# OpenDriveLab/OccNet

Measured on AMD Instinct MI355X. Metric: nuScenes samples/sec (6-cam 900x1600 -> 200x200x16 voxels), higher is better.
Workload: dtype f32 hot path (GEMM operands bf16x3-split, SCA value rows q16 block floating point) + bf16 backbone; 1 GPU; bevformer_base_occ forward: 6x(3x928x1600) images -> ResNet-50+FPN -> 4 BEVFormer layers (TSA+SCA+FFN) -> lifter + 2xConv3d decoder -> 200x200x16 voxels x (17 logits + 2 flow); history_frames=0, mode=infer, scope=e2e, input=resident-f32, samples_per_gpu=1, global_batch=1, parallelism=dp1, step_graph=False, linear_precision=bf16x3, backbone_dtype=bf16

## Files before the change

include/occnet_amd.h:

```cpp
#ifndef OCCNET_AMD_H_
#define OCCNET_AMD_H_

#include <stdint.h>

#ifdef __cplusplus
extern "C" {
#endif

#define OCC_OK 0
#define OCC_E_INVALID (-1)
#define OCC_E_LAUNCH (-2)
#define OCC_E_UNSUPPORTED (-3)

int occ_abi_version(void);
const char* occ_last_error(void);
int occ_selftest_fdiv_f32(const float* a, const float* d, float* q, int64_t n, void* stream);


int occ_ms_deform_attn_forward_f32(const float* value, const int64_t* spatial_shapes,
                                   const int64_t* level_start_index, const float* sampling_loc,
                                   const float* attn_weight, float* out, int B, int S, int M, int D,
                                   int L, int Lq, int P, int im2col_step, void* stream);

int occ_ms_deform_attn_backward_f32(const float* value, const int64_t* spatial_shapes,
// ... 121 lines not shown

int occ_sca_prep_forward_f32(const float* proj, int64_t proj_batch_stride, int proj_ld, const int64_t* row_to_query,
                             const float* ref_rb, const int64_t* spatial_shapes, float* loc, float* attn, int B,
                             int64_t R, int M, int L, int P, int Z, void* stream);
int occ_sca_prep_backward_f32(const float* grad_loc, const float* grad_attn, const float* attn,
                              const int64_t* query_to_rows, int Kq, const int64_t* spatial_shapes, float* dproj,
                              int proj_ld, int B, int64_t R, int64_t Q, int M, int L, int P, void* stream);

int occ_rows_gather_sum_f32(const float* x, int64_t x_batch_stride, const int64_t* index, int K, float* out, int B,
                            int64_t rows_out, int64_t rows_in, int F, void* stream);

int64_t occ_linear_wgrad_workspace_bytes(int M, int N, int K);
int occ_linear_wgrad_bf16x3_f32(const float* dy, int64_t lddy, const float* x, int64_t ldx, float* dw, float* db,
                                void* workspace, int64_t workspace_bytes, int M, int N, int K, void* stream);

int64_t occ_conv3d_wgrad_workspace_bytes(int B, int Z, int Y, int X, int Cin);
int occ_conv3d_wgrad_bf16x3_f32(const float* dy_pad, const float* x_pad, float* dw, void* workspace,
                                int64_t workspace_bytes, int B, int Z, int Y, int X, int Cin, void* stream);

int occ_bias_act_nhwc_bf16(void* x, const float* bias, const void* residual, int64_t rows, int C, int relu,
                           void* stream);

int64_t occ_bias_act_bwd_partial_floats(int64_t rows, int C);
int occ_bias_act_bwd_nhwc_bf16(const void* grad_y, const void* y, void* g, float* partial, float* bias_grad,
                               int64_t rows, int C, int relu, void* stream);

int occ_conv_bn_fold_fwd_f32(const float* weight, const float* gamma, const float* beta, const float* rstd,
                             const float* mean_rstd, float* w_folded, void* w_folded_bf16_nhwc, float* bias, int Cout,
                             int Cin, int KH, int KW, void* stream);
int occ_conv_bn_fold_bwd_f32(const void* grad_w_bf16, int64_t stride_o, int64_t stride_i, int64_t stride_h, int64_t stride_w,
                             const float* weight, const float* gamma, const float* rstd, const float* mean_rstd,
                             const float* grad_bias, float* grad_weight, float* grad_gamma, int Cout, int Cin, int KH, int KW,
                             void* stream);

unsigned occ_ln_dropout_hash(unsigned index, unsigned seed_lo, unsigned seed_hi);
int64_t occ_dropout_add_ln_bwd_partial_floats(int64_t rows, int C);
int occ_dropout_add_ln_fwd_f32(const float* x, const float* residual, const float* gamma, const float* beta, float eps,
                               float p_drop, uint64_t seed, float* z, float* y, float* stats, int64_t rows, int C,
                               void* stream);
int occ_dropout_add_ln_bwd_f32(const float* grad_y, const float* z, const float* stats, const float* gamma, float p_drop,
                               uint64_t seed, float* grad_x, float* grad_residual, float* partial, float* grad_gamma_beta,
                               int64_t rows, int C, void* stream);

int occ_value_proj_bf16_f32(int n_segments, const void* const* a, const int64_t* lda, const int64_t* rows,
                            const int64_t* rows_per_group, const int64_t* out_row0,
                            const float* const* group_bias, int bias_groups, const void* weight_packed,
                            float* out, int64_t ldo, int K, int N, int64_t out_group_rows, void* stream);
int occ_value_proj_bf16_f16pairs(int n_segments, const void* const* a, const int64_t* lda, const int64_t* rows,
                            const int64_t* rows_per_group, const int64_t* out_row0,
                            const float* const* group_bias, int bias_groups, const void* weight_packed,
                            void* out, int64_t ldo, int K, int N, int64_t out_group_rows, const float* out_scale,
                            void* stream);
int occ_value_proj_bf16_q16pairs(int n_segments, const void* const* a, const int64_t* lda, const int64_t* rows,
                            const int64_t* rows_per_group, const int64_t* out_row0,
                            const float* const* group_bias, int bias_groups, const void* weight_packed,
                            void* out, int64_t ldo, int K, int N, int64_t out_group_rows, const float* out_scale,
                            void* stream);

int occ_value_range_scale_bf16(int n_segments, const void* const* a, const int64_t* lda, const int64_t* rows, int K,
                               int n_planes, const float* row_l1, const float* bias_max, float* scale_out,
                               uint32_t* work, void* stream);
int occ_value_range_scale_from_amax(const uint32_t* amax8, int n_planes, const float* row_l1, const float* bias_max,
                                    float* scale_out, void* stream);

int occ_value_proj_bf16_planes(int n_segments, const void* const* a, const int64_t* lda, const int64_t* rows,
                               const int64_t* rows_per_group, const int64_t* out_row0,
                               const float* const* group_bias, int bias_groups, const void* weight_packed, void* out,
                               int out_f16, int64_t ldo, int K, int n_planes, int plane_cols, int64_t plane_stride,
                               int64_t out_group_rows, const float* out_scale, void* stream);

int occ_stem_conv7x7_pool_f32_bf16(const float* x, const void* weight_frag, const float* bias, void* out,
                                   int batch, int H, int W, void* stream);
int occ_stem_conv7x7_pool_u8_bf16(const uint8_t* x, const void* weight_frag, const float* bias, void* out,
                                  int batch, int Hs, int Ws, int H, int W, const float* mean,
                                  const float* std, int to_rgb, void* stream);

int occ_bias_relu_maxpool_nhwc_bf16(const void* y, const float* bias, void* out, int batch, int H, int W, int C,
                                    void* stream);

int occ_conv1x1_nhwc_bf16(const void* x, const void* weight, const float* bias, const void* residual,
                          void* out, int batch, int Hin, int Win, int Cin, int Cout, int stride, int relu,
                          int residual_upsample2, void* stream);

int occ_conv3x3_pack_weight_bf16(const float* weight, void* packed, int Cout, int Cin, void* stream);
int occ_conv3x3_nhwc_bf16(const void* x, const void* weight_packed, const float* bias, void* out, int batch,
                          int H, int W, int Cin, int Cout, int stride, int relu, void* stream);
int occ_conv3x3_nhwc_bf16_amax(const void* x, const void* weight_packed, const float* bias, void* out, int batch,
                               int H, int W, int Cin, int Cout, int stride, int relu, uint32_t* amax8, void* stream);
int occ_conv3x3_nhwc_bf16_variant(const void* x, const void* weight_packed, const float* bias, void* out, int batch,
                                  int H, int W, int Cin, int Cout, int stride, int relu, uint32_t* amax8, int variant,
                                  void* stream);

int occ_mfma_pack_b_frag_bf16(const float* weight, void* packed, int N, int K, void* stream);

int occ_bottleneck64_nhwc_bf16(const void* x, const void* w1_frag, const float* b1, const void* w2_frag,
                               const float* b2, const void* w3_frag, const float* b3, void* out, int batch,
                               int H, int W, int Cin, int downsample, void* stream);

#ifdef __cplusplus
}
#endif
#endif
```

occnet_amd/csrc/conv1x1_nhwc_bf16.hip:

```cpp
#include "common.h"

namespace occ {

typedef float f32x16 __attribute__((ext_vector_type(16)));
typedef __bf16 bf16x8 __attribute__((ext_vector_type(8)));


__device__ __forceinline__ float c1_bf16_to_f32(unsigned short h) { return __uint_as_float((unsigned)h << 16); }

template <int NT, int RT>
__global__ __launch_bounds__(256) void conv1x1_nhwc_bf16_kernel(
    const uint4* __restrict__ x, const uint4* __restrict__ w, const float* __restrict__ bias,
    const unsigned short* __restrict__ residual, unsigned short* __restrict__ out, long M, int N, int K,
    int Hin, int Win, int Hout, int Wout, int stride, int relu, int res_up) {
  constexpr int KC = 32, kCLD = KC * 2 + 16, PC = KC / 8;
  constexpr int BM = 32 * RT, BN = 128 * NT, WR = 32 * NT, OLD = BN + 4;
  constexpr int AP = BM * PC / 256;
  constexpr int A_BYTES = BM * kCLD;
  constexpr int STAGE_BYTES = 2 * A_BYTES, OUT_BYTES = 32 * OLD * 4;
  __shared__ __attribute__((aligned(16))) char lds[STAGE_BYTES > OUT_BYTES ? STAGE_BYTES : OUT_BYTES];
  const int tid = threadIdx.x, lane = tid & 63, wave = tid >> 6;
  const int vi = lane & 31, kb = lane >> 5;
  const long m0 = (long)blockIdx.x * BM;
  const int n0 = blockIdx.y * BN;
  const int KQ = K / 8;
  const int NT32 = N / 32;

  f32x16 acc[RT][NT];
#pragma unroll
  for (int rt = 0; rt < RT; ++rt)
#pragma unroll
    for (int t = 0; t < NT; ++t)
#pragma unroll
      for (int r = 0; r < 16; ++r) acc[rt][t][r] = 0.f;

  static_assert(AP >= 1 && AP <= 2 && NT <= 2, "staging register budget");
  long aofs[AP];
  int adst[AP];
#pragma unroll
  for (int ap = 0; ap < AP; ++ap) {
    const int j = tid + 256 * ap;
    const int row = j / PC, piece = j % PC;
    long m = m0 + row;
    if (m >= M) m = M - 1;
    long pix = m;
    if (stride != 1) {
      const long hw = (long)Hout * Wout;
      const long n = m / hw, rem = m % hw;
      const int yo = (int)(rem / Wout), xo = (int)(rem % Wout);
      pix = (n * Hin + (long)yo * stride) * Win + (long)xo * stride;
    }
    aofs[ap] = pix * KQ + piece;
    adst[ap] = row * kCLD + piece * 16;
  }
  const int nt0 = min((n0 + wave * WR) / 32, NT32 - 1), nt1 = min((n0 + wave * WR) / 32 + (NT - 1), NT32 - 1);
  const long wl0 = (long)nt0 * 64 + lane, wl1 = (long)nt1 * 64 + lane;
  uint4 va0_0, va1_0, va0_1, va1_1;
  uint4 wa0_0, wa1_0, wb0_0, wb1_0, wa0_1, wa1_1, wb0_1, wb1_1, wa0_2, wa1_2, wb0_2, wb1_2;
#define OCC_C1_ISSUE_A(S, K0)                                                                     \
  {                                                                                               \
    const long kq = (K0) / 8;                                                                     \
    va0_##S = x[aofs[0] + kq];                                                                    \
    if (AP > 1) va1_##S = x[aofs[AP > 1 ? 1 : 0] + kq];                                           \
  }
#define OCC_C1_ISSUE_W(S, K0)                                                                     \
  {                                                                                               \
    const long k0 = (long)((K0) / 16) * NT32 * 64, k1 = k0 + (long)NT32 * 64;                     \
    wa0_##S = w[k0 + wl0]; wb0_##S = w[k1 + wl0];                                                 \
    if (NT > 1) { wa1_##S = w[k0 + wl1]; wb1_##S = w[k1 + wl1]; }                                 \
  }
#define OCC_C1_STEP(SA, SW, SWN, BUF, K_NEXT)                                                     \
  {                                                                                               \
    char* sA = lds + (BUF) * A_BYTES;                                                             \
    *reinterpret_cast<uint4*>(sA + adst[0]) = va0_##SA;                                           \
    if (AP > 1) *reinterpret_cast<uint4*>(sA + adst[AP > 1 ? 1 : 0]) = va1_##SA;                  \
    __syncthreads();                 \
    OCC_C1_ISSUE_A(SA, K_NEXT)                                                                    \
    OCC_C1_ISSUE_W(SWN, K_NEXT)                                                                   \
    bf16x8 af[RT][2];                                                                             \
    _Pragma("unroll") for (int rt = 0; rt < RT; ++rt)                                             \
      _Pragma("unroll") for (int ks = 0; ks < 2; ++ks)                                            \
        af[rt][ks] = *reinterpret_cast<const bf16x8*>(sA + (rt * 32 + vi) * kCLD + ks * 32 + kb * 16); \
// ... 1 lines not shown
      acc[rt][0] = __builtin_amdgcn_mfma_f32_32x32x16_bf16(af[rt][0], __builtin_bit_cast(bf16x8, wa0_##SW), acc[rt][0], 0, 0, 0); \
      if (NT > 1) acc[rt][NT - 1] = __builtin_amdgcn_mfma_f32_32x32x16_bf16(af[rt][0], __builtin_bit_cast(bf16x8, wa1_##SW), acc[rt][NT - 1], 0, 0, 0); \
    }                                                                                             \
    _Pragma("unroll") for (int rt = 0; rt < RT; ++rt) {                                           \
      acc[rt][0] = __builtin_amdgcn_mfma_f32_32x32x16_bf16(af[rt][1], __builtin_bit_cast(bf16x8, wb0_##SW), acc[rt][0], 0, 0, 0); \
      if (NT > 1) acc[rt][NT - 1] = __builtin_amdgcn_mfma_f32_32x32x16_bf16(af[rt][1], __builtin_bit_cast(bf16x8, wb1_##SW), acc[rt][NT - 1], 0, 0, 0); \
    }                                                                                             \
  }

  const int NCHK = K / KC;
  const int rot = (int)((blockIdx.x * 5u + blockIdx.y * 3u) % (unsigned)NCHK);
#define OCC_C1_K(CI) ((((CI) < NCHK ? (CI) : NCHK - 1) + rot) % NCHK * KC)
  OCC_C1_ISSUE_A(0, OCC_C1_K(0))
  OCC_C1_ISSUE_W(0, OCC_C1_K(0))
  OCC_C1_ISSUE_A(1, OCC_C1_K(1))
  OCC_C1_ISSUE_W(1, OCC_C1_K(1))
  for (int ci = 0; ci < NCHK; ci += 6) {
    OCC_C1_STEP(0, 0, 2, 0, OCC_C1_K(ci + 2))
    if (ci + 1 < NCHK) OCC_C1_STEP(1, 1, 0, 1, OCC_C1_K(ci + 3))
    if (ci + 2 < NCHK) OCC_C1_STEP(0, 2, 1, 0, OCC_C1_K(ci + 4))
    if (ci + 3 < NCHK) OCC_C1_STEP(1, 0, 2, 1, OCC_C1_K(ci + 5))
    if (ci + 4 < NCHK) OCC_C1_STEP(0, 1, 0, 0, OCC_C1_K(ci + 6))
    if (ci + 5 < NCHK) OCC_C1_STEP(1, 2, 1, 1, OCC_C1_K(ci + 7))
  }
#undef OCC_C1_K
#undef OCC_C1_STEP
#undef OCC_C1_ISSUE_A
#undef OCC_C1_ISSUE_W

  const int c = lane * 4;
  const bool col_live = c < BN && n0 + c < N;
  float4 bv = make_float4(0.f, 0.f, 0.f, 0.f);
  if (col_live) bv = *reinterpret_cast<const float4*>(bias + n0 + c);
  float* sO = reinterpret_cast<float*>(lds);
#pragma unroll
  for (int rt = 0; rt < RT; ++rt) {
    __syncthreads();
#pragma unroll
    for (int t = 0; t < NT; ++t)
#pragma unroll
      for (int r = 0; r < 16; ++r)
        sO[((r & 3) + 8 * (r >> 2) + 4 * kb) * OLD + (wave * NT + t) * 32 + vi] = acc[rt][t][r];
    __syncthreads();
    uint2 rv[8];
#pragma unroll
    for (int rr = 0; rr < 8; ++rr) {
      long m = m0 + rt * 32 + wave * 8 + rr;
      if (m >= M) m = M - 1;
      rv[rr] = make_uint2(0u, 0u);
      if (residual != nullptr && col_live) {
        long rrow = m;
        if (res_up) {
          const long hw = (long)Hout * Wout;
          const long n = m / hw, rem = m - n * hw;
          const int yo = (int)(rem / Wout), xo = (int)(rem - (long)yo * Wout);
          rrow = (n * (Hout >> 1) + (yo >> 1)) * (Wout >> 1) + (xo >> 1);
        }
        rv[rr] = *reinterpret_cast<const uint2*>(residual + rrow * N + n0 + c);
      }
    }
#pragma unroll
    for (int rr = 0; rr < 8; ++rr) {
      const int row = wave * 8 + rr;
      const long m = m0 + rt * 32 + row;
      if (m < M && col_live) {
        float4 v = *reinterpret_cast<const float4*>(sO + row * OLD + c);
        v.x += bv.x; v.y += bv.y; v.z += bv.z; v.w += bv.w;
        v.x += c1_bf16_to_f32((unsigned short)(rv[rr].x & 0xffffu));
        v.y += c1_bf16_to_f32((unsigned short)(rv[rr].x >> 16));
        v.z += c1_bf16_to_f32((unsigned short)(rv[rr].y & 0xffffu));
        v.w += c1_bf16_to_f32((unsigned short)(rv[rr].y >> 16));
        if (relu) {
          v.x = fmaxf(v.x, 0.f); v.y = fmaxf(v.y, 0.f); v.z = fmaxf(v.z, 0.f); v.w = fmaxf(v.w, 0.f);
        }
        const uint2 o = make_uint2(pack_bf16x2_rne(v.x, v.y), pack_bf16x2_rne(v.z, v.w));
        *reinterpret_cast<uint2*>(out + m * N + n0 + c) = o;
      }
    }
  }
}

}

extern "C" int occ_conv1x1_nhwc_bf16(const void* x, const void* weight, const float* bias,
                                     const void* residual, void* out, int batch, int Hin, int Win,
                                     int Cin, int Cout, int stride, int relu, int residual_upsample2,
                                     void* stream) {
  using namespace occ;
  OCC_CHECK_ARG(x && weight && bias && out, "conv1x1_nhwc_bf16: null pointer argument");
  OCC_CHECK_ARG(batch > 0 && Hin > 0 && Win > 0 && Cin > 0 && Cout > 0 && stride > 0,
                "conv1x1_nhwc_bf16: bad dimension");
  if (Cin % 32 || Cout % 32) {
    set_error("conv1x1_nhwc_bf16: no kernel for Cin=%d Cout=%d (need Cin %% 32 == 0, Cout %% 32 == 0)", Cin,
              Cout);
    return OCC_E_UNSUPPORTED;
  }
  const int Hout = (Hin - 1) / stride + 1, Wout = (Win - 1) / stride + 1;
  OCC_CHECK_ARG(!residual_upsample2 || (residual && Hout % 2 == 0 && Wout % 2 == 0),
                "conv1x1_nhwc_bf16: an upsampled residual needs even output sizes (exact x2 nearest upsampling)");
  const long M = (long)batch * Hout * Wout;
  hipStream_t st = reinterpret_cast<hipStream_t>(stream);
#define OCC_C1_LAUNCH(NTT, RTT, BNN)                                                                \
  hipLaunchKernelGGL((conv1x1_nhwc_bf16_kernel<NTT, RTT>),                                          \
                     dim3((unsigned)((M + 32 * RTT - 1) / (32 * RTT)), (unsigned)((Cout + BNN - 1) / BNN)), \
                     dim3(256), 0, st, reinterpret_cast<const uint4*>(x),                           \
                     reinterpret_cast<const uint4*>(weight), bias,                                  \
                     reinterpret_cast<const unsigned short*>(residual),                             \
                     reinterpret_cast<unsigned short*>(out), M, Cout, Cin, Hin, Win, Hout, Wout, stride, relu,  \
                     residual_upsample2)
  if (Cout <= 128) OCC_C1_LAUNCH(1, 2, 128); else OCC_C1_LAUNCH(2, 2, 256);
#undef OCC_C1_LAUNCH
  OCC_CHECK_LAUNCH("conv1x1_nhwc_bf16");
  return OCC_OK;
}
```

occnet_amd/ext.py:

```python
import ctypes
import os

import torch

from . import _lib, cache_epoch
from ._lib import OccAmdError, OccAmdUnsupported, f32, i32, i64, ptr, stream_ptr


_TIMING = None
_TIMING_ONLY = None


def kernel_timing(enable=True):
    global _TIMING, _TIMING_ONLY
    _TIMING = {} if enable else None
    _TIMING_ONLY = None
    return _TIMING


def kernel_timing_only(names):
    global _TIMING_ONLY
    _TIMING_ONLY = None if names is None else set(names)


# ... 1330 lines not shown
    so, si, sh, sw = grad_w16.stride()
    with torch.cuda.device(weight.device):
        rc = _lib.lib().occ_conv_bn_fold_bwd_f32(ptr(grad_w16), i64(so), i64(si), i64(sh), i64(sw), ptr(weight), ptr(gamma),
                                                 ptr(rstd), ptr(mean_rstd), ptr(grad_bias), ptr(dW), ptr(dgamma), i32(O), i32(I),
                                                 i32(KH), i32(KW), stream_ptr(weight.device))
    _lib.check(rc, "conv_bn_fold_bwd")
    return dW, dgamma


def stem_pack_weight(weight):
    if tuple(weight.shape) != (64, 3, 7, 7):
        raise OccAmdUnsupported("stem_pack_weight: expected a (64, 3, 7, 7) weight")
    w2 = torch.zeros(64, 7, 8, 4, dtype=torch.float32, device=weight.device)
    w2[:, :, :7, :3] = weight.float().permute(0, 2, 3, 1)
    return mfma_pack_b_frag(w2.reshape(64, 224))


def stem_conv7x7_pool(x, weight_frag, bias):
    _need_cuda_f32("x", x)
    _need_cuda_f32("bias", bias)
    if x.dim() != 4 or x.shape[1] != 3 or not x.is_contiguous():
        raise OccAmdUnsupported("stem_conv7x7_pool: x must be a contiguous (N, 3, H, W) fp32 tensor")
    if weight_frag.numel() != 64 * 224 or bias.numel() != 64:
        raise OccAmdError("stem_conv7x7_pool: inconsistent shapes")
    N, _, H, W = x.shape
    Hc, Wc = (H - 1) // 2 + 1, (W - 1) // 2 + 1
    Hp, Wp = (Hc - 1) // 2 + 1, (Wc - 1) // 2 + 1
    out = torch.empty((N, 64, Hp, Wp), dtype=torch.bfloat16, device=x.device, memory_format=torch.channels_last)
    with torch.cuda.device(x.device), _timed('bb_stem7x7_pool'):
        rc = _lib.lib().occ_stem_conv7x7_pool_f32_bf16(ptr(x), ptr(weight_frag), ptr(bias), ptr(out), i32(N),
                                                       i32(H), i32(W), stream_ptr(x.device))
    _note_flops('bb_stem7x7_pool', 2.0 * N * Hc * Wc * 64 * 147)
    _lib.check(rc, "stem_conv7x7_pool")
    return out


def stem_conv7x7_pool_u8(x_u8, weight_frag, bias, mean, std, to_rgb=False, size_divisor=32):
    if not (x_u8.is_cuda and x_u8.dtype == torch.uint8 and x_u8.dim() == 4 and x_u8.shape[-1] == 3
            and x_u8.is_contiguous()):
        raise OccAmdUnsupported("stem_conv7x7_pool_u8: x must be a contiguous (N, H, W, 3) uint8 device tensor")
    _need_cuda_f32("bias", bias)
    if weight_frag.numel() != 64 * 224 or bias.numel() != 64:
        raise OccAmdError("stem_conv7x7_pool_u8: inconsistent shapes")
    N, Hs, Ws, _ = x_u8.shape
    d = int(size_divisor)
    H, W = (Hs + d - 1) // d * d, (Ws + d - 1) // d * d
    Hc, Wc = (H - 1) // 2 + 1, (W - 1) // 2 + 1
    Hp, Wp = (Hc - 1) // 2 + 1, (Wc - 1) // 2 + 1
    out = torch.empty((N, 64, Hp, Wp), dtype=torch.bfloat16, device=x_u8.device, memory_format=torch.channels_last)
    mean_c = (f32 * 3)(*[float(v) for v in mean])
    std_c = (f32 * 3)(*[float(v) for v in std])
    with torch.cuda.device(x_u8.device):
        rc = _lib.lib().occ_stem_conv7x7_pool_u8_bf16(ptr(x_u8), ptr(weight_frag), ptr(bias), ptr(out), i32(N),
                                                      i32(Hs), i32(Ws), i32(H), i32(W), mean_c, std_c,
                                                      i32(1 if to_rgb else 0), stream_ptr(x_u8.device))
    _lib.check(rc, "stem_conv7x7_pool_u8")
    return out, (H, W)


def bias_relu_maxpool_nhwc(y, bias):
    if not (y.is_cuda and y.dtype == torch.bfloat16 and y.dim() == 4
            and y.is_contiguous(memory_format=torch.channels_last)):
        raise OccAmdUnsupported("bias_relu_maxpool_nhwc: y must be a channels_last bfloat16 device tensor")
    _need_cuda_f32("bias", bias)
    N, C, H, W = y.shape
    if bias.numel() != C:
        raise OccAmdError("bias_relu_maxpool_nhwc: bias must have C entries")
    out = torch.empty((N, C, (H - 1) // 2 + 1, (W - 1) // 2 + 1), dtype=torch.bfloat16, device=y.device,
                      memory_format=torch.channels_last)
    with torch.cuda.device(y.device):
        rc = _lib.lib().occ_bias_relu_maxpool_nhwc_bf16(ptr(y), ptr(bias), ptr(out), i32(N), i32(H), i32(W),
                                                        i32(C), stream_ptr(y.device))
    _lib.check(rc, "bias_relu_maxpool_nhwc")
    return out


def conv1x1_pack_weight(weight2d):
    cout, cin = weight2d.shape
    if cin % 32 or cout % 32:
        raise OccAmdUnsupported("conv1x1_pack_weight: Cin and Cout must be multiples of 32")
    return mfma_pack_b_frag(weight2d.float().contiguous())


def conv1x1_nhwc(x, weight_frag, bias, residual=None, relu=False, stride=1, residual_upsample2=False):
    if not (x.is_cuda and x.dtype == torch.bfloat16 and x.dim() == 4
            and x.is_contiguous(memory_format=torch.channels_last)):
        raise OccAmdUnsupported("conv1x1_nhwc: x must be a channels_last bfloat16 device tensor")
    _need_cuda_f32("bias", bias)
    N, Cin, H, W = x.shape
    Cout = bias.numel()
    if not (weight_frag.dtype == torch.int16 and weight_frag.dim() == 1 and weight_frag.is_contiguous()
            and weight_frag.numel() == Cout * Cin):
        raise OccAmdError("conv1x1_nhwc: weight must come from conv1x1_pack_weight (Cout*Cin bf16, fragment order)")
    s = int(stride)
    Ho, Wo = (H - 1) // s + 1, (W - 1) // s + 1
    out = torch.empty((N, Cout, Ho, Wo), dtype=torch.bfloat16, device=x.device,
                      memory_format=torch.channels_last)
    want = (N, Cout, Ho // 2, Wo // 2) if residual_upsample2 else tuple(out.shape)
    if residual_upsample2 and (residual is None or Ho % 2 or Wo % 2):
        raise OccAmdUnsupported("conv1x1_nhwc: an upsampled residual needs even output sizes")
    if residual is not None and not (residual.dtype == torch.bfloat16 and tuple(residual.shape) == want and
                                     residual.is_contiguous(memory_format=torch.channels_last)):
        raise OccAmdUnsupported("conv1x1_nhwc: residual must match the output (channels_last bfloat16)")
    with torch.cuda.device(x.device), _timed('bb_conv1x1'):
        rc = _lib.lib().occ_conv1x1_nhwc_bf16(ptr(x), ptr(weight_frag), ptr(bias), ptr(residual), ptr(out),
                                              i32(N), i32(H), i32(W), i32(Cin), i32(Cout), i32(s),
                                              i32(1 if relu else 0), i32(1 if residual_upsample2 else 0),
                                              stream_ptr(x.device))
    _note_flops('bb_conv1x1', 2.0 * N * Ho * Wo * Cin * Cout)
    _lib.check(rc, "conv1x1_nhwc")
    return out


def mfma_pack_b_frag(weight2d):
    _need_cuda_f32("weight", weight2d)
    if weight2d.dim() != 2:
        raise OccAmdError("mfma_pack_b_frag: expected a (N, K) matrix")
    weight2d = weight2d.contiguous()
    n, k = weight2d.shape
    packed = torch.empty(n * k, dtype=torch.int16, device=weight2d.device)
    with torch.cuda.device(weight2d.device):
        rc = _lib.lib().occ_mfma_pack_b_frag_bf16(ptr(weight2d), ptr(packed), i32(n), i32(k),
                                                  stream_ptr(weight2d.device))
    _lib.check(rc, "mfma_pack_b_frag")
    return packed


def bottleneck64_pack(w1, b1, w2, b2, w3, b3, wds=None, bds=None):
    w1 = w1.float().reshape(w1.shape[0], -1)
    w3 = w3.float().reshape(w3.shape[0], -1)
    if tuple(w2.shape) != (64, 64, 3, 3) or w1.shape[0] != 64 or tuple(w3.shape) != (256, 64):
        raise OccAmdUnsupported("bottleneck64_pack: only 64 mid / 256 output channels")
    ds = wds is not None
    cin = w1.shape[1]
    if (ds and cin != 64) or (not ds and cin != 256):
        raise OccAmdUnsupported("bottleneck64_pack: Cin must be 256 (identity) or 64 (projection)")
    w2m = w2.float().permute(0, 2, 3, 1).reshape(64, 9 * 64)
    b3 = b3.float()
    if ds:
        w3 = torch.cat([w3, wds.float().reshape(256, 64)], dim=1)
        b3 = b3 + bds.float()
    return dict(w1=mfma_pack_b_frag(w1), b1=b1.float().contiguous(), w2=mfma_pack_b_frag(w2m),
                b2=b2.float().contiguous(), w3=mfma_pack_b_frag(w3), b3=b3.contiguous(), cin=cin, ds=ds)


def bottleneck64_nhwc(x, pack):
    if not (x.is_cuda and x.dtype == torch.bfloat16 and x.dim() == 4
            and x.is_contiguous(memory_format=torch.channels_last)):
        raise OccAmdUnsupported("bottleneck64_nhwc: x must be a channels_last bfloat16 device tensor")
    N, Cin, H, W = x.shape
    if Cin != pack['cin']:
        raise OccAmdError("bottleneck64_nhwc: x has %d channels, the pack was built for %d" % (Cin, pack['cin']))
    out = torch.empty((N, 256, H, W), dtype=torch.bfloat16, device=x.device, memory_format=torch.channels_last)
    with torch.cuda.device(x.device), _timed('bb_bottleneck64'):
        rc = _lib.lib().occ_bottleneck64_nhwc_bf16(ptr(x), ptr(pack['w1']), ptr(pack['b1']), ptr(pack['w2']),
                                                   ptr(pack['b2']), ptr(pack['w3']), ptr(pack['b3']), ptr(out),
                                                   i32(N), i32(H), i32(W), i32(Cin), i32(1 if pack['ds'] else 0),
                                                   stream_ptr(x.device))
    _note_flops('bb_bottleneck64', 2.0 * N * H * W * (Cin * 64 + 9 * 64 * 64 + 64 * 256 + (Cin * 256 if pack['ds'] else 0)))
    _lib.check(rc, "bottleneck64_nhwc")
    return out


def conv3x3_pack_weight(weight):
    _need_cuda_f32("weight", weight)
    if weight.dim() != 4 or tuple(weight.shape[2:]) != (3, 3):
        raise OccAmdError("conv3x3_pack_weight: expected a (Cout, Cin, 3, 3) weight")
    cout, cin = weight.shape[:2]
    packed = torch.empty(weight.numel(), dtype=torch.int16, device=weight.device)
    with torch.cuda.device(weight.device):
        rc = _lib.lib().occ_conv3x3_pack_weight_bf16(ptr(weight), ptr(packed), i32(cout), i32(cin),
                                                     stream_ptr(weight.device))
    _lib.check(rc, "conv3x3_pack_weight")
    return packed


def conv3x3_nhwc(x, w_packed, bias, cout, relu=False, stride=1, amax=None, variant=None):
    if not (x.is_cuda and x.dtype == torch.bfloat16 and x.dim() == 4
            and x.is_contiguous(memory_format=torch.channels_last)):
        raise OccAmdUnsupported("conv3x3_nhwc: x must be a channels_last bfloat16 device tensor")
    _need_cuda_f32("bias", bias)
    N, Cin, H, W = x.shape
    if w_packed.numel() != cout * Cin * 9 or bias.numel() != cout:
        raise OccAmdError("conv3x3_nhwc: inconsistent shapes")
    st = int(stride)
    if st not in (1, 2):
        raise OccAmdUnsupported("conv3x3_nhwc: stride must be 1 or 2")
    if amax is not None and not (amax.is_cuda and amax.dtype == torch.int32 and amax.numel() == 8 and amax.is_contiguous()):
        raise OccAmdError("conv3x3_nhwc: amax must be 8 contiguous int32 device words")
    out = torch.empty((N, cout, (H - 1) // st + 1, (W - 1) // st + 1), dtype=torch.bfloat16, device=x.device,
                      memory_format=torch.channels_last)
# ... 18 lines not shown
```

tools_dev/conv_probe.py:

```python
import os, sys
sys.path.insert(0, os.path.join(os.path.dirname(os.path.abspath(__file__)), ".."))
import torch
from occnet_amd import ext


def timeit(fn, iters=20):
    for _ in range(3):
        fn()
    a, b = torch.cuda.Event(enable_timing=True), torch.cuda.Event(enable_timing=True)
    torch.cuda.synchronize(); a.record()
    for _ in range(iters):
        fn()
    b.record(); torch.cuda.synchronize()
    return a.elapsed_time(b) * 1e3 / iters


def main(which):
    g = torch.Generator().manual_seed(0)
    N = 6
    mk = lambda *s: (torch.randn(*s, generator=g) * 0.05).cuda()
    act = lambda c, h, w: torch.randn(N, c, h, w, generator=g).cuda().to(torch.bfloat16).contiguous(
        memory_format=torch.channels_last)
    if 'c3' in which or 'c3v' in which:
        def variants(s, cout):
            if 'c3v' not in which:
                return (None,)
            vs = (12, 13, 14, 16, 18, 22, 23, 24) if s == 1 else (12, 13, 22)
            return (None,) + tuple(v for v in vs if cout % (128 * (v // 10)) == 0)
        for (cin, cout, h, w, s) in [(128, 128, 232, 400, 2), (128, 128, 116, 200, 1), (256, 256, 116, 200, 2),
                                     (256, 256, 58, 100, 1), (512, 512, 58, 100, 2), (512, 512, 29, 50, 1),
                                     (256, 256, 116, 200, 1), (256, 256, 29, 50, 1),
                                     (256, 256, 29, 50, 2)]:
            x, wp, b = act(cin, h, w), ext.conv3x3_pack_weight(mk(cout, cin, 3, 3)), mk(cout)
            vs = variants(s, cout)
            rounds = 5 if len(vs) > 1 else 1
            times = {v: [] for v in vs}
            for _ in range(rounds):
                for v in vs:
                    times[v].append(timeit(lambda: ext.conv3x3_nhwc(x, wp, b, cout, relu=True, stride=s, variant=v)))
            for v in vs:
                us = sorted(times[v])[rounds // 2]
                ho, wo = (h - 1) // s + 1, (w - 1) // s + 1
                fl = 2.0 * N * ho * wo * cout * cin * 9
                tag = 'auto' if v is None else f'v{v}'
                print(f"conv3x3 {cin:4d}->{cout:4d} {h:3d}x{w:3d} s{s} {tag:4s}: {us:7.1f} us  {fl / us * 1e-6:6.1f} TF/s")
    if 'c1' in which:
        for (cin, cout, h, w, s, res) in [(256, 128, 232, 400, 1, 0), (128, 512, 116, 200, 1, 1),
                                          (512, 128, 116, 200, 1, 0), (256, 512, 232, 400, 2, 0),
                                          (512, 256, 116, 200, 1, 0), (256, 1024, 58, 100, 1, 1),
                                          (1024, 256, 58, 100, 1, 0), (512, 1024, 116, 200, 2, 0),
                                          (1024, 512, 58, 100, 1, 0), (512, 2048, 29, 50, 1, 1),
                                          (2048, 512, 29, 50, 1, 0), (1024, 2048, 58, 100, 2, 0),
                                          (512, 256, 116, 200, 1, 0), (1024, 256, 58, 100, 1, 0),
                                          (2048, 256, 29, 50, 1, 0)]:
            x, wp, b = act(cin, h, w), ext.conv1x1_pack_weight(mk(cout, cin)), mk(cout)
            ho, wo = (h - 1) // s + 1, (w - 1) // s + 1
            r = act(cout, ho, wo) if res else None
            us = timeit(lambda: ext.conv1x1_nhwc(x, wp, b, residual=r, relu=True, stride=s))
            fl = 2.0 * N * ho * wo * cout * cin
            mb = N * (ho * wo * (cin + cout * (2 if res else 1))) * 2 / 1e6
            print(f"conv1x1 {cin:4d}->{cout:4d} {h:3d}x{w:3d} s{s} res{res}: {us:7.1f} us  {fl / us * 1e-6:6.1f} TF/s  "
                  f"{mb / us:5.2f} TB/s")


def vp():
    g = torch.Generator().manual_seed(0)
    w = (torch.randn(256, 256, generator=g) / 16).cuda()
    gb = torch.randn(6, 256, generator=g).cuda()
    total = 23200 + 5800 + 1450 + 375
    out = torch.empty(6 * total, 256, device='cuda')
    hws = (23200, 5800, 1450, 375)
    a_list = [torch.randn(6 * hw, 256, generator=g).cuda().to(torch.bfloat16) for hw in hws]
    gb4 = gb.unsqueeze(0).repeat(4, 1, 1).contiguous()
    starts = [0, 23200, 29000, 30450]
    us = timeit(lambda: ext.value_proj_bf16(a_list, w, gb4, out, rows_per_group=list(hws), out_group_rows=total,
                                            out_row0=starts))
    mb = 6 * total * 256 * (2 + 4) / 1e6
    print(f"value_proj_bf16 all levels M={6 * total}: {us:7.1f} us  {mb / us:5.2f} TB/s")
    x = torch.randn(6 * total, 256, generator=g).cuda()
    b = torch.randn(256, generator=g).cuda()
    us = timeit(lambda: ext.linear(x, w, b))
    print(f"linear bf16x3 f32 in M={6 * total}: {us:7.1f} us")


if __name__ == '__main__':
    if 'vp' in sys.argv[1:]:
        vp()
    main(sys.argv[1:] or ['c3', 'c1'])
```

Baseline: 185.8 samples/s.

## Add activation-resident conv1x1 kernel that keeps input rows in LDS across all output columns

Adds a new conv1x1 NHWC bf16 kernel for Cin 128/256/512 that loads a block of input rows into LDS once, then streams pre-packed weights from global memory through a register ring while looping over output-column passes. The epilogue fuses bias, residual (including x2-upsampled residual) and ReLU through per-wave LDS scratch. It is enabled by default for eligible shapes and uses an L2-friendly block-to-column mapping. The aim is to stop re-reading activations once per column tile, at the cost of more LDS, higher register pressure and weight re-reads per row block.

```diff
diff --git a/include/occnet_amd.h b/include/occnet_amd.h
--- a/include/occnet_amd.h
+++ b/include/occnet_amd.h
@@ -227,6 +227,10 @@
                           void* out, int batch, int Hin, int Win, int Cin, int Cout, int stride, int relu,
                           int residual_upsample2, void* stream);
 
+int occ_conv1x1_nhwc_bf16_variant(const void* x, const void* weight, const float* bias, const void* residual,
+                                  void* out, int batch, int Hin, int Win, int Cin, int Cout, int stride, int relu,
+                                  int residual_upsample2, int variant, void* stream);
+
 int occ_conv3x3_pack_weight_bf16(const float* weight, void* packed, int Cout, int Cin, void* stream);
 int occ_conv3x3_nhwc_bf16(const void* x, const void* weight_packed, const float* bias, void* out, int batch,
                           int H, int W, int Cin, int Cout, int stride, int relu, void* stream);
diff --git a/occnet_amd/csrc/conv1x1_nhwc_bf16.hip b/occnet_amd/csrc/conv1x1_nhwc_bf16.hip
--- a/occnet_amd/csrc/conv1x1_nhwc_bf16.hip
+++ b/occnet_amd/csrc/conv1x1_nhwc_bf16.hip
@@ -1,3 +1,4 @@
+#include <cstdlib>
 #include "common.h"
 
 namespace occ {
@@ -165,10 +166,16 @@
 
 }
 
-extern "C" int occ_conv1x1_nhwc_bf16(const void* x, const void* weight, const float* bias,
-                                     const void* residual, void* out, int batch, int Hin, int Win,
-                                     int Cin, int Cout, int stride, int relu, int residual_upsample2,
-                                     void* stream) {
+namespace occ {
+int conv1x1_resident_tile(int Cin, int Cout, long M, long in_pixels, int rt);
+int conv1x1_resident_launch(const void* x, const void* weight, const float* bias, const void* residual, void* out,
+                            long M, int Hin, int Win, int Hout, int Wout, int Cin, int Cout, int stride, int relu,
+                            int residual_upsample2, int rt, int ncb_force, hipStream_t st);
+}
+
+static int conv1x1_nhwc_bf16_launch(const void* x, const void* weight, const float* bias, const void* residual,
+                                    void* out, int batch, int Hin, int Win, int Cin, int Cout, int stride, int relu,
+                                    int residual_upsample2, int variant, void* stream) {
   using namespace occ;
   OCC_CHECK_ARG(x && weight && bias && out, "conv1x1_nhwc_bf16: null pointer argument");
   OCC_CHECK_ARG(batch > 0 && Hin > 0 && Win > 0 && Cin > 0 && Cout > 0 && stride > 0,
@@ -182,7 +189,26 @@
   OCC_CHECK_ARG(!residual_upsample2 || (residual && Hout % 2 == 0 && Wout % 2 == 0),
                 "conv1x1_nhwc_bf16: an upsampled residual needs even output sizes (exact x2 nearest upsampling)");
   const long M = (long)batch * Hout * Wout;
+  const long in_pixels = (long)batch * Hin * Win;
   hipStream_t st = reinterpret_cast<hipStream_t>(stream);
+  static const bool resident_on = [] { const char* e = getenv("OCC_CONV1X1_RESIDENT"); return !(e && e[0] == '0'); }();
+  int rt = 0, ncb_force = 0;
+  if (variant == 0) {
+    if (resident_on && M >= 512) rt = conv1x1_resident_tile(Cin, Cout, M, in_pixels, 0);
+  } else if (variant != 1) {
+    const int v = variant % 100;
+    ncb_force = variant / 100;
+    const int want = v == 2 && ncb_force == 0 ? 0 : v == 22 ? 2 : v == 24 ? 4 : -1;
+    rt = variant < 0 || want < 0 ? 0 : conv1x1_resident_tile(Cin, Cout, M, in_pixels, want);
+    if (rt == 0) {
+      set_error("conv1x1_nhwc_bf16: no variant %d for Cin=%d Cout=%d (1 = tiled; 2, 22, 24 = activation-resident: Cin 128 / "
+                "256 / 512, Cout %% 128 == 0, Cout <= 4096; 22 only Cin 512)", variant, Cin, Cout);
+      return OCC_E_UNSUPPORTED;
+    }
+  }
+  if (rt != 0)
+    return conv1x1_resident_launch(x, weight, bias, residual, out, M, Hin, Win, Hout, Wout, Cin, Cout, stride, relu,
+                                   residual_upsample2, rt, ncb_force, st);
 #define OCC_C1_LAUNCH(NTT, RTT, BNN)                                                                \
   hipLaunchKernelGGL((conv1x1_nhwc_bf16_kernel<NTT, RTT>),                                          \
                      dim3((unsigned)((M + 32 * RTT - 1) / (32 * RTT)), (unsigned)((Cout + BNN - 1) / BNN)), \
@@ -196,3 +222,19 @@
   OCC_CHECK_LAUNCH("conv1x1_nhwc_bf16");
   return OCC_OK;
 }
+
+extern "C" int occ_conv1x1_nhwc_bf16(const void* x, const void* weight, const float* bias,
+                                     const void* residual, void* out, int batch, int Hin, int Win,
+                                     int Cin, int Cout, int stride, int relu, int residual_upsample2,
+                                     void* stream) {
+  return conv1x1_nhwc_bf16_launch(x, weight, bias, residual, out, batch, Hin, Win, Cin, Cout, stride, relu,
+                                  residual_upsample2, 0, stream);
+}
+
+extern "C" int occ_conv1x1_nhwc_bf16_variant(const void* x, const void* weight, const float* bias,
+                                             const void* residual, void* out, int batch, int Hin, int Win,
+                                             int Cin, int Cout, int stride, int relu, int residual_upsample2,
+                                             int variant, void* stream) {
+  return conv1x1_nhwc_bf16_launch(x, weight, bias, residual, out, batch, Hin, Win, Cin, Cout, stride, relu,
+                                  residual_upsample2, variant, stream);
+}
diff --git a/occnet_amd/csrc/conv1x1_resident_bf16.hip b/occnet_amd/csrc/conv1x1_resident_bf16.hip
--- /dev/null
+++ b/occnet_amd/csrc/conv1x1_resident_bf16.hip
@@ -0,0 +1,271 @@
+#include <cstdlib>
+#include "common.h"
+
+namespace occ {
+
+typedef float f32x16 __attribute__((ext_vector_type(16)));
+typedef __bf16 bf16x8 __attribute__((ext_vector_type(8)));
+typedef __attribute__((address_space(3))) void* c1r_lds_ptr_t;
+
+constexpr int kC1rPitch = 80, kC1rScratch = 32 * kC1rPitch;
+
+__device__ __forceinline__ float c1r_lo(unsigned v) { return __uint_as_float(v << 16); }
+__device__ __forceinline__ float c1r_hi(unsigned v) { return __uint_as_float(v & 0xffff0000u); }
+
+__device__ __forceinline__ int up2_row(int m, int Hout, int Wout) {
+  const unsigned hw = (unsigned)(Hout * Wout);
+  const unsigned n = (unsigned)m / hw, rem = (unsigned)m - n * hw;
+  const unsigned yo = rem / (unsigned)Wout, xo = rem - yo * (unsigned)Wout;
+  return (int)((n * (unsigned)(Hout >> 1) + (yo >> 1)) * (unsigned)(Wout >> 1) + (xo >> 1));
+}
+
+constexpr int c1r_lds_bytes(int K, int RT, int bias_cols) { return 32 * RT * K * 2 + 4 * kC1rScratch + bias_cols * 4; }
+
+template <int K, int RT, int NTW, int RES, int MINB, int RD>
+__global__ __launch_bounds__(256, MINB) void conv1x1_resident_kernel(
+    const uint4* __restrict__ x, const uint4* __restrict__ wp, const float* __restrict__ bias,
+    const unsigned short* __restrict__ residual, unsigned short* __restrict__ out, int M, int N, int Hin, int Win,
+    int Hout, int Wout, int stride, int relu, int nrb, int ncb, int ppb) {
+  extern __shared__ __attribute__((aligned(16))) char clds[];
+  constexpr int BM = 32 * RT, PCS = K / 8, PITCH = K * 2, KS = K / 16;
+  constexpr int MASK = (PCS < 32 ? PCS : 32) - 1;
+  constexpr int RPI = 64 / PCS;
+  constexpr int NINST = BM / RPI / 4;
+  constexpr int TILE_BYTES = BM * PITCH;
+  constexpr int NTILES = RT * NTW;
+  static_assert(PCS <= 64 && KS % 4 == 0 && NTILES >= 2 && RT % 2 == 0 && RD >= 1 && RD <= NTILES, "tile geometry");
+  const int tid = threadIdx.x, lane = tid & 63, wave = tid >> 6;
+  const int vi = lane & 31, kb = lane >> 5;
+  int rb = (int)blockIdx.x, cb = 0;
+  if (ncb > 1) {
+    const int id = (int)blockIdx.x, grp = id / (8 * ncb), within = id % (8 * ncb);
+    rb = grp * 8 + (within & 7);
+    cb = within >> 3;
+  }
+  if (rb >= nrb) return;
+  const int m0 = rb * BM;
+  const int NT32 = N / 32;
+
+#pragma unroll
+  for (int j = 0; j < NINST; ++j) {
+    const int inst = wave * NINST + j;
+    const int r = inst * RPI + lane / PCS, slot = lane % PCS;
+    int m = m0 + r;
+    if (m >= M) m = M - 1;
+    int pix = m;
+    if (stride != 1) {
+      const unsigned hw = (unsigned)(Hout * Wout);
+      const unsigned n = (unsigned)m / hw, rem = (unsigned)m - n * hw;
+      const unsigned yo = rem / (unsigned)Wout, xo = rem - yo * (unsigned)Wout;
+      pix = (int)((n * (unsigned)Hin + yo * (unsigned)stride) * (unsigned)Win + xo * (unsigned)stride);
+    }
+    __builtin_amdgcn_global_load_lds(x + (long)pix * PCS + (slot ^ (r & MASK)), (c1r_lds_ptr_t)(clds + inst * 1024), 16, 0, 0);
+  }
+
+  occ_u32x4 w[4][NTW];
+  const __amdgpu_buffer_rsrc_t wr = uniform_rsrc(wp, (unsigned)K * (unsigned)N * 2u);
+  const int wv = (wave * NTW * 64 + lane) * 16;
+  const int kstep_bytes = NT32 * 1024;
+#define OCC_C1R_LOAD(SLOT, PASS, KSTEP)                                                            \
+  {                                                                                               \
+    const int so = (KSTEP) * kstep_bytes + (PASS) * (4 * NTW * 1024);                             \
+    _Pragma("unroll") for (int t = 0; t < NTW; ++t)                                               \
+      w[SLOT][t] = __builtin_amdgcn_raw_buffer_load_b128(wr, wv + t * 1024, so, 0);               \
+  }
+  const int p0 = cb * ppb;
+  float* const sbias = reinterpret_cast<float*>(clds + TILE_BYTES + 4 * kC1rScratch);
+  for (int i = tid; i < ppb * (32 * NTW); i += 256)
+    *reinterpret_cast<float4*>(sbias + 4 * i) = *reinterpret_cast<const float4*>(bias + p0 * (128 * NTW) + 4 * i);
+  OCC_C1R_LOAD(0, p0, 0)
+  OCC_C1R_LOAD(1, p0, 1)
+  OCC_C1R_LOAD(2, p0, 2)
+  __syncthreads();
+
+  char* const scratch = clds + TILE_BYTES + wave * kC1rScratch;
+
+  bf16x8 af[2][RT];
+  unsigned abase = (unsigned)(vi * PITCH + ((kb ^ vi) & MASK) * 16);
+#define OCC_C1R_AFRAG(BUF, KSTEP)                                                                  \
+  {                                                                                               \
+    asm volatile("" : "+v"(abase));                                                               \
+    const char* ap = clds + (abase ^ (unsigned)((KSTEP) * 32));                                   \
+    _Pragma("unroll") for (int rt = 0; rt < RT; ++rt)                                             \
+      af[BUF][rt] = *reinterpret_cast<const bf16x8*>(ap + rt * (32 * PITCH));                     \
+  }
+#define OCC_C1R_RES(DST, NW, RTI, TI)                                                              \
+  {                                                                                               \
+    _Pragma("unroll") for (int j = 0; j < 2; ++j) {                                               \
+      int m = m0 + (RTI) * 32 + (rlane >> 2) + 16 * j;                                            \
+      if (m >= M) m = M - 1;                                                                      \
+      if (RES == 2) m = up2_row(m, Hout, Wout);                                                   \
+      DST[j] = *reinterpret_cast<const uint4*>(residual + (long)m * N + (NW) + (TI) * 32 + (rlane & 3) * 8); \
+    }                                                                                             \
+  }
+  uint4 rq[RD][2];
+  int rlane = lane;
+  if (RES) {
+    const int nw0 = p0 * (128 * NTW) + wave * (32 * NTW);
+#pragma unroll
+    for (int i = 0; i < RD; ++i) OCC_C1R_RES(rq[i], nw0, i / NTW, i % NTW)
+  }
+  OCC_C1R_AFRAG(0, 0)
+#pragma unroll 1
+  for (int p = p0; p < p0 + ppb; ++p) {
+    const int nw = p * (128 * NTW) + wave * (32 * NTW);
+    int elane = lane;
+    asm volatile("" : "+v"(elane));
+    f32x16 acc[RT][NTW];
+#pragma unroll
+    for (int t = 0; t < NTW; ++t)
+#pragma unroll
+      for (int q = 0; q < 4; ++q) {
+        const float4 c0 = *reinterpret_cast<const float4*>(sbias + (nw - p0 * (128 * NTW)) + t * 32 + 8 * q + 4 * kb);
+#pragma unroll
+        for (int rt = 0; rt < RT; ++rt) {
+          acc[rt][t][4 * q + 0] = c0.x;
+          acc[rt][t][4 * q + 1] = c0.y;
+          acc[rt][t][4 * q + 2] = c0.z;
+          acc[rt][t][4 * q + 3] = c0.w;
+        }
+      }
+    const int pn = p + 1 < p0 + ppb ? p + 1 : p;
+#pragma unroll
+    for (int ks = 0; ks < KS; ++ks) {
+      if (ks + 3 < KS) OCC_C1R_LOAD((ks + 3) & 3, p, ks + 3)
+      else OCC_C1R_LOAD((ks + 3) & 3, pn, ks + 3 - KS)
+      OCC_C1R_AFRAG((ks + 1) & 1, (ks + 1) & (KS - 1))
+#pragma unroll
+      for (int rt = 0; rt < RT; ++rt)
+#pragma unroll
+        for (int t = 0; t < NTW; ++t)
+          acc[rt][t] = __builtin_amdgcn_mfma_f32_32x32x16_bf16(__builtin_bit_cast(bf16x8, w[ks & 3][t]), af[ks & 1][rt],
+                                                               acc[rt][t], 0, 0, 0);
+      if (NTILES >= 4) {
+        constexpr int MQ = NTILES / 4;
+        __builtin_amdgcn_sched_group_barrier(0x008, MQ, 0);
+        __builtin_amdgcn_sched_group_barrier(0x020, 1, 0);
+        __builtin_amdgcn_sched_group_barrier(0x008, MQ, 0);
+        __builtin_amdgcn_sched_group_barrier(0x100, RT / 2, 0);
+        __builtin_amdgcn_sched_group_barrier(0x008, MQ, 0);
+        if (NTW > 1) __builtin_amdgcn_sched_group_barrier(0x020, 1, 0);
+        __builtin_amdgcn_sched_group_barrier(0x008, MQ, 0);
+        __builtin_amdgcn_sched_group_barrier(0x100, RT / 2, 0);
+      } else {
+        __builtin_amdgcn_sched_group_barrier(0x008, 1, 0);
+        __builtin_amdgcn_sched_group_barrier(0x020, 1, 0);
+        __builtin_amdgcn_sched_group_barrier(0x100, 1, 0);
+        __builtin_amdgcn_sched_group_barrier(0x008, 1, 0);
+        __builtin_amdgcn_sched_group_barrier(0x100, 1, 0);
+      }
+    }
+
+    const int erow = elane >> 2, epiece = elane & 3;
+#pragma unroll
+    for (int rt = 0; rt < RT; ++rt) {
+#pragma unroll
+      for (int t = 0; t < NTW; ++t) {
+        const int e = rt * NTW + t;
+        if (RES) {
+          const uint4 r0 = rq[0][0], r1 = rq[0][1];
+#pragma unroll
+          for (int i = 0; i + 1 < RD; ++i) { rq[i][0] = rq[i + 1][0]; rq[i][1] = rq[i + 1][1]; }
+          asm volatile("" : "+v"(rlane));
+          if (e + RD < NTILES) OCC_C1R_RES(rq[RD - 1], nw, (e + RD) / NTW, (e + RD) % NTW)
+          else if (p + 1 < p0 + ppb) OCC_C1R_RES(rq[RD - 1], nw + 128 * NTW, (e + RD - NTILES) / NTW, (e + RD - NTILES) % NTW)
+          *reinterpret_cast<uint4*>(scratch + erow * kC1rPitch + epiece * 16) = r0;
+          *reinterpret_cast<uint4*>(scratch + (erow + 16) * kC1rPitch + epiece * 16) = r1;
+          wave_lds_sync();
+        }
+#pragma unroll
+        for (int q = 0; q < 4; ++q) {
+          char* const sp = scratch + vi * kC1rPitch + 16 * q + 8 * kb;
+          float v0 = acc[rt][t][4 * q + 0], v1 = acc[rt][t][4 * q + 1], v2 = acc[rt][t][4 * q + 2],
+                v3 = acc[rt][t][4 * q + 3];
+          if (RES) {
+            const uint2 r = *reinterpret_cast<const uint2*>(sp);
+            v0 += c1r_lo(r.x); v1 += c1r_hi(r.x); v2 += c1r_lo(r.y); v3 += c1r_hi(r.y);
+          }
+          if (relu) { v0 = fmaxf(v0, 0.f); v1 = fmaxf(v1, 0.f); v2 = fmaxf(v2, 0.f); v3 = fmaxf(v3, 0.f); }
+          *reinterpret_cast<uint2*>(sp) = make_uint2(pack_bf16x2_rne(v0, v1), pack_bf16x2_rne(v2, v3));
+        }
+        wave_lds_sync();
+#pragma unroll
+        for (int j = 0; j < 2; ++j) {
+          const int row = erow + 16 * j;
+          const int m = m0 + rt * 32 + row;
+          const uint4 v = *reinterpret_cast<const uint4*>(scratch + row * kC1rPitch + epiece * 16);
+          if (m < M) *reinterpret_cast<uint4*>(out + (long)m * N + nw + t * 32 + epiece * 8) = v;
+        }
+        wave_lds_sync();
+      }
+    }
+  }
+#undef OCC_C1R_RES
+#undef OCC_C1R_AFRAG
+#undef OCC_C1R_LOAD
+}
+
+int conv1x1_resident_tile(int Cin, int Cout, long M, long in_pixels, int rt) {
+  if ((Cin != 128 && Cin != 256 && Cin != 512) || Cout % 128 || Cout > 4096) return 0;
+  if (M >= (1L << 30) || in_pixels >= (1L << 30)) return 0;
+  if (rt == 0) rt = Cin == 512 ? 2 : 4;
+  if (rt == 4) return 4;
+  if (rt == 2 && Cin == 512) return 2;
+  return 0;
+}
+
+int conv1x1_resident_launch(const void* x, const void* weight, const float* bias, const void* residual, void* out,
+                            long M, int Hin, int Win, int Hout, int Wout, int Cin, int Cout, int stride, int relu,
+                            int residual_upsample2, int rt, int ncb_force, hipStream_t st) {
+  const int ntw = Cout % 256 == 0 ? 2 : 1;
+  const int np = Cout / (128 * ntw);
+  const int nrb = (int)((M + 32 * rt - 1) / (32 * rt));
+  const long want_blocks = Cin == 128 ? 2048 : 1024;
+  int ncb = np;
+  for (int d = 1; d <= np; ++d)
+    if (np % d == 0 && (long)nrb * d >= want_blocks) { ncb = d; break; }
+  if (ncb_force > 0) {
+    if (np % ncb_force) {
+      set_error("conv1x1_nhwc_bf16: no variant with %d column blocks for %d passes", ncb_force, np);
+      return OCC_E_UNSUPPORTED;
+    }
+    ncb = ncb_force;
+  }
+  const int ppb = np / ncb;
+  const unsigned grid = ncb > 1 ? (unsigned)((nrb + 7) / 8 * 8 * ncb) : (unsigned)nrb;
+  hipError_t e = hipSuccess;
+#define OCC_C1R_GO(KK, RTT, NTT, RR, MINB, RDD)                                                          \
+  {                                                                                               \
+    auto kern = conv1x1_resident_kernel<KK, RTT, NTT, RR, MINB, RR ? RDD : 1>;                                  \
+    const int lds = c1r_lds_bytes(KK, RTT, ppb * 128 * NTT);                                                \
+    e = hipFuncSetAttribute(reinterpret_cast<const void*>(kern), hipFuncAttributeMaxDynamicSharedMemorySize, lds); \
+    if (e == hipSuccess)                                                                          \
+      hipLaunchKernelGGL(kern, dim3(grid), dim3(256), lds, st, reinterpret_cast<const uint4*>(x),  \
+                         reinterpret_cast<const uint4*>(weight), bias,                            \
+                         reinterpret_cast<const unsigned short*>(residual),                       \
+                         reinterpret_cast<unsigned short*>(out), (int)M, Cout, Hin, Win, Hout, Wout, stride, relu, nrb, \
+                         ncb, ppb);                                                               \
+  }
+#define OCC_C1R_RES_(KK, RTT, NTT, MINB, RDD)                                                       \
+  {                                                                                               \
+    if (residual && residual_upsample2) OCC_C1R_GO(KK, RTT, NTT, 2, MINB, RDD)                    \
+    else if (residual) OCC_C1R_GO(KK, RTT, NTT, 1, MINB, RDD)                                     \
+    else OCC_C1R_GO(KK, RTT, NTT, 0, MINB, RDD)                                                   \
+  }
+#define OCC_C1R_NT_(KK, RTT, MINB, RD2, RD1) { if (ntw == 2) OCC_C1R_RES_(KK, RTT, 2, MINB, RD2) else OCC_C1R_RES_(KK, RTT, 1, MINB, RD1) }
+  if (Cin == 128) OCC_C1R_NT_(128, 4, 2, 6, 4)
+  else if (Cin == 256) OCC_C1R_NT_(256, 4, 2, 4, 4)
+  else if (rt == 2) OCC_C1R_NT_(512, 2, 2, 4, 2)
+  else OCC_C1R_NT_(512, 4, 1, 8, 4)
+#undef OCC_C1R_NT_
+#undef OCC_C1R_RES_
+#undef OCC_C1R_GO
+  if (e != hipSuccess) {
+    set_error("conv1x1_nhwc_bf16: hipFuncSetAttribute failed: %s", hipGetErrorString(e));
+    return OCC_E_LAUNCH;
+  }
+  OCC_CHECK_LAUNCH("conv1x1_nhwc_bf16 (resident)");
+  return OCC_OK;
+}
+
+}
diff --git a/occnet_amd/ext.py b/occnet_amd/ext.py
--- a/occnet_amd/ext.py
+++ b/occnet_amd/ext.py
@@ -1436,7 +1436,7 @@
     return mfma_pack_b_frag(weight2d.float().contiguous())
 
 
-def conv1x1_nhwc(x, weight_frag, bias, residual=None, relu=False, stride=1, residual_upsample2=False):
+def conv1x1_nhwc(x, weight_frag, bias, residual=None, relu=False, stride=1, residual_upsample2=False, variant=None):
     if not (x.is_cuda and x.dtype == torch.bfloat16 and x.dim() == 4
             and x.is_contiguous(memory_format=torch.channels_last)):
         raise OccAmdUnsupported("conv1x1_nhwc: x must be a channels_last bfloat16 device tensor")
@@ -1457,10 +1457,16 @@
                                      residual.is_contiguous(memory_format=torch.channels_last)):
         raise OccAmdUnsupported("conv1x1_nhwc: residual must match the output (channels_last bfloat16)")
     with torch.cuda.device(x.device), _timed('bb_conv1x1'):
-        rc = _lib.lib().occ_conv1x1_nhwc_bf16(ptr(x), ptr(weight_frag), ptr(bias), ptr(residual), ptr(out),
-                                              i32(N), i32(H), i32(W), i32(Cin), i32(Cout), i32(s),
-                                              i32(1 if relu else 0), i32(1 if residual_upsample2 else 0),
-                                              stream_ptr(x.device))
+        if variant is None:
+            rc = _lib.lib().occ_conv1x1_nhwc_bf16(ptr(x), ptr(weight_frag), ptr(bias), ptr(residual), ptr(out),
+                                                  i32(N), i32(H), i32(W), i32(Cin), i32(Cout), i32(s),
+                                                  i32(1 if relu else 0), i32(1 if residual_upsample2 else 0),
+                                                  stream_ptr(x.device))
+        else:
+            rc = _lib.lib().occ_conv1x1_nhwc_bf16_variant(ptr(x), ptr(weight_frag), ptr(bias), ptr(residual), ptr(out),
+                                                          i32(N), i32(H), i32(W), i32(Cin), i32(Cout), i32(s),
+                                                          i32(1 if relu else 0), i32(1 if residual_upsample2 else 0),
+                                                          i32(int(variant)), stream_ptr(x.device))
     _note_flops('bb_conv1x1', 2.0 * N * Ho * Wo * Cin * Cout)
     _lib.check(rc, "conv1x1_nhwc")
     return out
diff --git a/tools_dev/conv1x1_pmc_table.py b/tools_dev/conv1x1_pmc_table.py
--- /dev/null
+++ b/tools_dev/conv1x1_pmc_table.py
@@ -0,0 +1,35 @@
+#!/usr/bin/env python
+import collections
+import csv
+import re
+import sys
+
+
+def main():
+    acc = collections.defaultdict(lambda: collections.defaultdict(lambda: [0, 0.0]))
+    for path in sys.argv[1:]:
+        with open(path) as f:
+            for row in csv.DictReader(f):
+                name = row['Kernel_Name']
+                if 'conv1x1' not in name:
+                    continue
+                m = re.search(r'(conv1x1_\w+)<([^>]*)>', name)
+                k = (f"{m.group(1)}<{m.group(2)}>" if m else name[:60], int(row['Grid_Size']) // 256)
+                a = acc[k][row['Counter_Name']]
+                a[0] += 1
+                a[1] += float(row['Counter_Value'])
+    print("# per-launch means.  kcyc = SQ_BUSY_CYCLES / 32 (XCD x SE instances); MfmaUtil = SQ_VALU_MFMA_BUSY_CYCLES / (kcyc * 1024")
+    print("# SIMDs); TA = TA_BUSY_avr / kcyc; wait = SQ_WAIT_INST_ANY / SQ_WAVE_CYCLES; FETCH / WRITE_SIZE in MB as reported (KB units)")
+    print(f"{'kernel<K, RT, NTW, RES, MINB, RD> | tiled <NT, RT>':58s} {'blocks':>7s} {'n':>4s} {'kcyc':>8s} {'Mfma':>6s} {'TA':>6s} "
+          f"{'wait':>6s} {'FETCH_MB':>9s} {'WRITE_MB':>9s}")
+    for k, c in sorted(acc.items()):
+        def mean(n):
+            return c[n][1] / c[n][0] if n in c and c[n][0] else float('nan')
+        dur = mean('SQ_BUSY_CYCLES') / 32
+        print(f"{k[0][:58]:58s} {k[1]:7d} {max(v[0] for v in c.values()):4d} {dur / 1e3:8.1f} "
+              f"{mean('SQ_VALU_MFMA_BUSY_CYCLES') / (dur * 1024):6.3f} {mean('TA_BUSY_avr') / dur:6.3f} "
+              f"{mean('SQ_WAIT_INST_ANY') / mean('SQ_WAVE_CYCLES'):6.3f} {mean('FETCH_SIZE') / 1e3:9.1f} {mean('WRITE_SIZE') / 1e3:9.1f}")
+
+
+if __name__ == '__main__':
+    main()
diff --git a/tools_dev/conv_probe.py b/tools_dev/conv_probe.py
--- a/tools_dev/conv_probe.py
+++ b/tools_dev/conv_probe.py
@@ -44,23 +44,44 @@
                 fl = 2.0 * N * ho * wo * cout * cin * 9
                 tag = 'auto' if v is None else f'v{v}'
                 print(f"conv3x3 {cin:4d}->{cout:4d} {h:3d}x{w:3d} s{s} {tag:4s}: {us:7.1f} us  {fl / us * 1e-6:6.1f} TF/s")
-    if 'c1' in which:
-        for (cin, cout, h, w, s, res) in [(256, 128, 232, 400, 1, 0), (128, 512, 116, 200, 1, 1),
-                                          (512, 128, 116, 200, 1, 0), (256, 512, 232, 400, 2, 0),
-                                          (512, 256, 116, 200, 1, 0), (256, 1024, 58, 100, 1, 1),
-                                          (1024, 256, 58, 100, 1, 0), (512, 1024, 116, 200, 2, 0),
-                                          (1024, 512, 58, 100, 1, 0), (512, 2048, 29, 50, 1, 1),
-                                          (2048, 512, 29, 50, 1, 0), (1024, 2048, 58, 100, 2, 0),
-                                          (512, 256, 116, 200, 1, 0), (1024, 256, 58, 100, 1, 0),
-                                          (2048, 256, 29, 50, 1, 0)]:
+    if 'c1' in which or 'c1v' in which or 'c1x' in which:
+        def variants(cin, cout, res):
+            if 'c1v' not in which and 'c1x' not in which:
+                return (None,)
+            if cin > 512:
+                return (None, 1)
+            vs = [None, 1, 2]
+            if 'c1x' in which:
+                np_ = cout // (256 if cout % 256 == 0 else 128)
+                tiles = (24, 22) if cin == 512 else (24,)
+                vs += [100 * d + t for t in tiles for d in range(1, np_ + 1) if np_ % d == 0]
+            return tuple(vs)
+        for (cin, cout, h, w, s, res, relu) in [(256, 128, 232, 400, 1, 0, 1), (128, 512, 116, 200, 1, 1, 1),
+                                                (512, 128, 116, 200, 1, 0, 1), (256, 512, 232, 400, 2, 0, 0),
+                                                (512, 256, 116, 200, 1, 0, 1), (256, 1024, 58, 100, 1, 1, 1),
+                                                (1024, 256, 58, 100, 1, 0, 1), (512, 1024, 116, 200, 2, 0, 0),
+                                                (1024, 512, 58, 100, 1, 0, 1), (512, 2048, 29, 50, 1, 1, 1),
+                                                (2048, 512, 29, 50, 1, 0, 1), (1024, 2048, 58, 100, 2, 0, 0),
+                                                (512, 256, 116, 200, 1, 2, 0), (1024, 256, 58, 100, 1, 2, 0),
+                                                (2048, 256, 29, 50, 1, 0, 0)]:
             x, wp, b = act(cin, h, w), ext.conv1x1_pack_weight(mk(cout, cin)), mk(cout)
             ho, wo = (h - 1) // s + 1, (w - 1) // s + 1
-            r = act(cout, ho, wo) if res else None
-            us = timeit(lambda: ext.conv1x1_nhwc(x, wp, b, residual=r, relu=True, stride=s))
+            r = act(cout, ho, wo) if res == 1 else act(cout, ho // 2, wo // 2) if res == 2 else None
+            vs = variants(cin, cout, res)
+            rounds = 5 if len(vs) > 1 else 1
+            times = {v: [] for v in vs}
+            for _ in range(rounds):
+                for v in vs:
+                    times[v].append(timeit(lambda: ext.conv1x1_nhwc(x, wp, b, residual=r, relu=bool(relu), stride=s,
+                                                                    residual_upsample2=res == 2, variant=v)))
             fl = 2.0 * N * ho * wo * cout * cin
-            mb = N * (ho * wo * (cin + cout * (2 if res else 1))) * 2 / 1e6
-            print(f"conv1x1 {cin:4d}->{cout:4d} {h:3d}x{w:3d} s{s} res{res}: {us:7.1f} us  {fl / us * 1e-6:6.1f} TF/s  "
-                  f"{mb / us:5.2f} TB/s")
+            mb = N * (ho * wo * (cin + cout * (2 if res == 1 else 1.25 if res == 2 else 1))) * 2 / 1e6
+            for v in vs:
+                t = sorted(times[v])
+                us = t[rounds // 2]
+                tag = 'auto' if v is None else f'v{v}'
+                print(f"conv1x1 {cin:4d}->{cout:4d} {h:3d}x{w:3d} s{s} res{res} {tag:5s}: {us:7.1f} us "
+                      f"[{t[0]:6.1f} - {t[-1]:6.1f}]  {fl / us * 1e-6:6.1f} TF/s  {mb / us:5.2f} TB/s", flush=True)
 
 
 def vp():
```

New measurement: 190.1 samples/s, median of 6. +2.3%, better.
